# nishitbohra/RoViT-KAN-Interpretable-Vision-Transformer-for-Rose-Disease-Severity-Estimation

Measured on AMD Instinct MI355X. Metric: images/sec fwd+bwd, DeiT-Tiny+KAN 224^2, batch 256 per GPU, higher is better.
Workload: dtype bf16; 1 GPU; full RoViT-KAN (DeiT-Tiny + KAN + 3 heads) stage 4, train mode, batch 256/GPU, 224x224x3 randn images, random-init weights; step=fwd + JointLoss + bwd + grad all-reduce + clip_grad_norm(1.0) + AdamW, global_batch=256, parallelism=dp1, grad_buckets=2, rccl_world=0

## Files before the change

### include/rovit_hip.h

```cpp
#ifndef ROVIT_HIP_H
#define ROVIT_HIP_H

#include <stddef.h>
#include <stdint.h>

#ifdef __cplusplus
extern "C" {
#endif

typedef void* rovit_stream_t;

enum {
  ROVIT_OK = 0,
  ROVIT_ERR_SHAPE = -1,
  ROVIT_ERR_ALIGN = -2,
  ROVIT_ERR_NULL = -3,
  ROVIT_ERR_LAUNCH = -4
};

enum { ROVIT_ACT_NONE = 0, ROVIT_ACT_RELU = 1, ROVIT_ACT_SIGMOID3 = 2 };
enum { ROVIT_LIN_RELU = 1, ROVIT_LIN_CLAMP10 = 2 };
enum { ROVIT_EPI_BF16 = 0, ROVIT_EPI_GELU = 1, ROVIT_EPI_RESID = 2, ROVIT_EPI_MUL = 3, ROVIT_EPI_PATCH = 4 };
enum { ROVIT_GEMM_TILED_192 = 0x100, ROVIT_GEMM_TILED_96 = 0x200 };

// ... 133 lines not shown
                        float* rstd_out, float eps, rovit_stream_t stream);
size_t rovit_mlp_stream_bytes(void);
int rovit_mlp_prepare_stream(const void* w1f, const void* w2, void* wstream, rovit_stream_t stream);
int rovit_mlp_fused_fwd(const void* xhat2, const void* wstream, const float* b1, const float* b2, void* act, void* dact, float* X,
                        void* xhat_out, float* rstd_out, float eps, int M, int act_rows, rovit_stream_t stream);
int rovit_mlp_prepare_stream_tail(const void* w1f, const void* w2, const void* wproj, const void* wqkv_next, void* wstream,
                                  rovit_stream_t stream);
int rovit_block_tail_fwd(const void* o, const void* wstream, const float* bp, const float* b1, const float* b2, float* X, void* xhat2,
                         float* rstd2, void* act, void* dact, void* xhat_out, float* rstd_out, const float* bq_next, void* qkv_next,
                         float eps, int M, int act_rows, rovit_stream_t stream);
int rovit_mlp_fused_bwd(const void* dY, const void* wstream_bwd, const void* dact, void* dpre, const void* xhat2, const float* rstd2,
                        float* dX, void* dXb, int M, rovit_stream_t stream);
int rovit_mlp_prepare_stream_bwd(const void* w2T, const void* w1T, const void* wqkvT_next, void* wstream, rovit_stream_t stream);
int rovit_block_bwd_fused(const void* dqkv, const void* xhat1, const float* rstd1, const void* xmid_in, void* xout, const void* wstream_bwd,
                          const void* dact, void* dpre, const void* xhat2, const float* rstd2, void* dXb, int M, rovit_stream_t stream);
int rovit_gemm_ln_bwd(const void* dY, int ldy, const void* W, int ldw, int M, int K, const void* xhat, const float* rstd, float* dX,
                      const void* dXb_in, void* dXb, rovit_stream_t stream);
int rovit_wgrad_splits(int M, int N, int K);
size_t rovit_wgrad_workspace_bytes(int N, int K, int splits);
int rovit_wgrad(const void* dY, int ldy, const void* A, int lda, int M, int N, int K, int splits, int patch_tokens, float* ws,
                rovit_stream_t stream);
int rovit_wgrad_multi(const void* const* dY, const int* ldy, const void* const* A, const int* lda, const int* N, const int* K,
                      float* const* ws, int n, int M, int splits, rovit_stream_t stream);
int rovit_wgrad_multi_ex(const void* const* dY, const int* ldy, const void* const* A, const int* lda, const int* N, const int* K,
                         float* const* ws, const int* a_blk, const int* y_blk, int n, int M, int splits, rovit_stream_t stream);
int rovit_wgrad_reduce(const float* ws, int splits, int N, int K, const float* gamma, const float* beta, const float* W,
                       float* dW, float* db, float* dgamma, float* dbeta, float* g_scratch, rovit_stream_t stream);
int rovit_attention_fwd(const void* qkv, void* out, float* lse2, int batch, int tokens, int heads, int head_dim, float scale,
                        rovit_stream_t stream);
int rovit_attention_probs(const void* qkv, float* probs, int batch, int tokens, int heads, int head_dim, float scale,
                          rovit_stream_t stream);
int rovit_attention_bwd(const void* qkv, const void* out, const float* lse2, const void* dout, void* dqkv, int batch, int tokens,
// ... 363 lines not shown
```

### rovit-kan-interpretable-vision-transformer-for-rose-disease-severity-estimation_amd/csrc/common.h

```cpp
#pragma once
#include <hip/hip_runtime.h>
#include <stdint.h>
#include <stdio.h>

#include "../../include/rovit_hip.h"

typedef __bf16 bf16;
typedef __attribute__((ext_vector_type(8))) __bf16 bf16x8;
typedef __attribute__((ext_vector_type(4))) __bf16 bf16x4;
typedef __attribute__((ext_vector_type(4))) float f32x4;
typedef __attribute__((ext_vector_type(2))) float f32x2;

#define ROVIT_WAVE 64

void rovit_set_error(const char* fmt, ...);

#define ROVIT_CHECK_ARG(cond, code, ...)        \
  do {                                          \
    if (!(cond)) {                              \
      rovit_set_error(__VA_ARGS__);             \
      return (code);                            \
    }                                           \
  } while (0)

// ... 22 lines not shown
  ROVIT_KNOB_MLP_DBG = 7,
  ROVIT_KNOB_MLP_SCHEDULE = 8,
  ROVIT_KNOB_MLP_RPW = 9,
  ROVIT_KNOB_WGRAD_TILE = 10,
  ROVIT_KNOB_WGRAD_WGS = 11,
  ROVIT_KNOB_KAN_MFMA_NS = 12,
  ROVIT_KNOB_KDMA = 13,
  ROVIT_KNOB_SKIP_DX_FP32_STORE = 15,
  ROVIT_KNOB_SIDE_PRIORITY = 16,
  ROVIT_KNOB_PROJ_DGRAD_CUS = 17,
  ROVIT_KNOB_TAIL_WAVES = 18,
  ROVIT_KNOB_FWD_STAGGER = 19,
  ROVIT_KNOB_ATTN_FWD3 = 20,
  ROVIT_KNOB_GRADCAM_RECOMPUTE = 21,
  ROVIT_KNOB_SKIP_WGRAD_REDUCE = 14,
  ROVIT_KNOB_COUNT = 32
};
#ifdef ROVIT_DEV
extern int g_rovit_knob[ROVIT_KNOB_COUNT];
extern bool g_rovit_knob_set[ROVIT_KNOB_COUNT];
#define ROVIT_KNOB(id, dflt) (g_rovit_knob_set[id] ? g_rovit_knob[id] : (dflt))
#else
#define ROVIT_KNOB(id, dflt) (dflt)
#endif

#ifdef __HIPCC__

__device__ __forceinline__ f32x4 mfma16(bf16x8 a, bf16x8 b, f32x4 c) {
  return __builtin_amdgcn_mfma_f32_16x16x32_bf16(a, b, c, 0, 0, 0);
}
// ... 103 lines not shown
                       const int* targets, float* logits, int* chosen, float* dfeat, const float* wqkv, void* wt, int batch,
                       rovit_stream_t stream);
int rovit_gradcam_cam(const void* dqkv, const void* wt, const void* xhat1, const float* gamma, const float* beta, float* g, double* spart,
                      float* act, float* grad, float* cam, int batch, rovit_stream_t stream);
int rovit_gather_token_rows(const float* img_tokens, const float* base_tokens, int n_img, int base_shared, const int* seq_img, const int* src,
                            float* X, int n_seq, int tokens, rovit_stream_t stream);
int rovit_gradcam_wt(const float* wqkv, void* wt, rovit_stream_t stream);
int rovit_cls_tail_fwd(const void* o, float* X, const void* wproj, const float* bproj, const void* wfc1, const float* bfc1, const void* wfc2,
                       const float* bfc2, const float* gamma, const float* beta, void* xhat2, float* rstd2, void* act, void* dact, float* feat,
                       float* xhat_cls, float* rstd_cls, int rows, int tokens, float eps, rovit_stream_t stream);
int rovit_cls_tail_bwd(const float* dfeat, const float* xhat_cls, const float* rstd_cls, const float* gamma, const void* wfc2, const void* wfc1,
                       const void* wproj, const void* dact, const void* xhat2, const float* rstd2, void* xin, void* dpre, void* xmid, void* dO,
                       int rows, int tokens, rovit_stream_t stream);
int rovit_attention_bwd_rows(const void* qkv, const void* out, const float* lse2, const void* dout, int dout_rows, void* dqkv, int batch,
                             int tokens, int heads, int head_dim, float scale, rovit_stream_t stream);
int rovit_gemm_ln_bwd_cls(const void* dY, int ldy, const void* W, int ldw, int M, int K, const void* xhat, const float* rstd,
                          const void* dXb_in, int cls_step, void* dXb, rovit_stream_t stream);
struct RovitWgradDesc { const void* dY; int ldy; const void* A; int lda; int N, K; float* ws; int a_blk, y_blk; };
int rovit_wgrad_batch(const RovitWgradDesc* descs, int n, int M, int splits, rovit_stream_t stream);

struct RovitReduceDesc {
  const float* ws; int splits, N, K;
  const float* gamma; const float* beta; const float* W;
  float* dW; float* db; float* dgamma; float* dbeta; float* g_scratch;
};
int rovit_mlp_stream_prep_blocks(const void* prep_base, size_t blk0, size_t stride, size_t off_w1, size_t off_w2, size_t off_out,
                                 size_t off_wp, int bwd, size_t off_wq_next, int depth, rovit_stream_t stream, bool gelu_tables = true);
constexpr int ROVIT_REDUCE_BATCH = 4;
int rovit_wgrad_reduce_batch(const RovitReduceDesc* descs, int n, rovit_stream_t stream);
```

### rovit-kan-interpretable-vision-transformer-for-rose-disease-severity-estimation_amd/csrc/gemm.hip

```cpp
#include <cstdlib>
#include <type_traits>
#include "common.h"

#ifdef ROVIT_DEV
#define GEMM_DBG(g, bit) ((g).dbg & (bit))
#define GEMM_SET_DBG(g, v) (g).dbg = (v)
#else
#define GEMM_DBG(g, bit) (false)
#define GEMM_SET_DBG(g, v) ((void)0)
#endif

namespace {

inline bool set_max_lds(const void* fn, size_t bytes) { return rovit_set_max_lds(fn, bytes); }

constexpr int BK = 64;
constexpr int LDS_STRIDE = BK + 16;

enum { EPI_BF16 = 0, EPI_GELU = 1, EPI_RESID = 2, EPI_MUL = 3, EPI_PATCH = 4, EPI_RESID_LN = 5, EPI_LNBWD = 6,
       EPI_PATCH_IMG = 7 };

struct GemmArgs {
  const bf16* A; int lda;
  const bf16* W; int ldw;
// ... 1497 lines not shown
  ROVIT_CHECK_ARG(descs && n >= 1 && n <= WG_MAXPROB && M > 0 && splits > 0, ROVIT_ERR_SHAPE, "wgrad_batch: bad arguments");
  WgradArgs g{};
  g.nprob = n;
  for (int j = 0; j < n; ++j) {
    const RovitWgradDesc& d = descs[j];
    ROVIT_CHECK_ARG(d.dY && d.A && d.ws, ROVIT_ERR_NULL, "wgrad_batch: null pointer");
    ROVIT_CHECK_ARG(d.N % 96 == 0 && d.K % 192 == 0, ROVIT_ERR_SHAPE, "wgrad_batch: unsupported shape N=%d K=%d", d.N, d.K);
    ROVIT_CHECK_ARG(d.ldy % 8 == 0 && d.lda % 8 == 0 && rovit_aligned16(d.dY) && rovit_aligned16(d.A), ROVIT_ERR_ALIGN, "wgrad_batch: alignment");
    ROVIT_CHECK_ARG(!(d.a_blk && d.K % 32) && !(d.y_blk && d.N % 32), ROVIT_ERR_SHAPE, "wgrad_batch: chunk-major operands need 32-column chunks");
    g.p[j] = WgradProb{(const bf16*)d.dY, d.ldy, (const bf16*)d.A, d.lda, d.N, d.K, d.ws, d.ws + (size_t)splits * d.N * d.K, 0, 0, d.a_blk, d.y_blk};
  }
  g.M = M;
  g.splits = splits;
  g.rows_per_split = ((M + splits - 1) / splits + WG_MSTEP - 1) / WG_MSTEP * WG_MSTEP;
  GEMM_SET_DBG(g, ROVIT_KNOB(ROVIT_KNOB_GEMM_DBG, 0) >> 4);
  if (n == 1 && g.p[0].K % 96 == 0) launch_wgrad<96, 96>(g, (hipStream_t)stream);
  else {
    for (int j = 0; j < n; ++j) ROVIT_CHECK_ARG(descs[j].N % 192 == 0 && descs[j].K % 192 == 0, ROVIT_ERR_SHAPE, "wgrad_batch: N, K %% 192 for 192-wide tiles");
    launch_wgrad<192, 192, 4>(g, (hipStream_t)stream);
  }
  ROVIT_CHECK_LAUNCH("wgrad_kernel (batch)");
  return ROVIT_OK;
}

extern "C" int rovit_wgrad_multi(const void* const* dY, const int* ldy, const void* const* A, const int* lda, const int* N, const int* K,
                                 float* const* ws, int n, int M, int splits, rovit_stream_t stream) {
  ROVIT_CHECK_ARG(dY && ldy && A && lda && N && K && ws && n >= 1 && n <= WG_MAXPROB, ROVIT_ERR_NULL, "wgrad_multi: bad arguments");
  RovitWgradDesc d[WG_MAXPROB];
  for (int j = 0; j < n; ++j) d[j] = {dY[j], ldy[j], A[j], lda[j], N[j], K[j], ws[j]};
  return rovit_wgrad_batch(d, n, M, splits, stream);
}
// ... 59 lines not shown
  GemmArgs g{};
  g.A = (const bf16*)A; g.lda = lda; g.W = (const bf16*)W; g.ldw = ldw; g.M = M; g.N = 192; g.K = K; g.bias = bias;
  g.xres = X; g.ldx = 192; g.out = (bf16*)xhat_out; g.ldo = 192; g.rstd_out = rstd_out; g.eps = eps; GEMM_SET_DBG(g, ROVIT_KNOB(ROVIT_KNOB_GEMM_DBG, 0));
  if (K == 192) return launch_ws<6, 1, 64>(g, EPI_RESID_LN, (hipStream_t)stream);
  if (kdma_enabled() && xhat_out && K == 576) return launch_kdma<18, EPI_RESID_LN>(g, (hipStream_t)stream);
  if (K == 576) return launch_ws<9, 2, 32>(g, EPI_RESID_LN, (hipStream_t)stream);
  return launch_ws<12, 2, 32>(g, EPI_RESID_LN, (hipStream_t)stream);
}

static int gemm_ln_bwd_impl(const void* dY, int ldy, const void* W, int ldw, int M, int K, const void* xhat, const float* rstd,
                            float* dX, const void* dXb_in, int cls_step, void* dXb, rovit_stream_t stream);
extern "C" int rovit_gemm_ln_bwd(const void* dY, int ldy, const void* W, int ldw, int M, int K, const void* xhat, const float* rstd,
                                 float* dX, const void* dXb_in, void* dXb, rovit_stream_t stream) {
  return gemm_ln_bwd_impl(dY, ldy, W, ldw, M, K, xhat, rstd, dX, dXb_in, 0, dXb, stream);
}
int rovit_gemm_ln_bwd_cls(const void* dY, int ldy, const void* W, int ldw, int M, int K, const void* xhat, const float* rstd,
                          const void* dXb_in, int cls_step, void* dXb, rovit_stream_t stream) {
  ROVIT_CHECK_ARG(dXb_in && cls_step > 0, ROVIT_ERR_NULL, "gemm_ln_bwd_cls: needs the bf16 incoming gradient and a row step");
  return gemm_ln_bwd_impl(dY, ldy, W, ldw, M, K, xhat, rstd, nullptr, dXb_in, cls_step, dXb, stream);
}
static int gemm_ln_bwd_impl(const void* dY, int ldy, const void* W, int ldw, int M, int K, const void* xhat, const float* rstd,
                            float* dX, const void* dXb_in, int cls_step, void* dXb, rovit_stream_t stream) {
  ROVIT_CHECK_ARG(dY && W && xhat && rstd && (dX || dXb_in) && dXb, ROVIT_ERR_NULL, "gemm_ln_bwd: null pointer");
  ROVIT_CHECK_ARG(rovit_aligned16(dXb_in) && rovit_aligned16(dXb), ROVIT_ERR_ALIGN, "gemm_ln_bwd: alignment");
  ROVIT_CHECK_ARG(M > 0 && (K == 192 || K == 576 || K == 768), ROVIT_ERR_SHAPE, "gemm_ln_bwd: K must be 192/576/768 (got %d)", K);
  ROVIT_CHECK_ARG(ldy % 8 == 0 && ldw % 8 == 0 && rovit_aligned16(dY) && rovit_aligned16(W) && rovit_aligned16(dX), ROVIT_ERR_ALIGN,
                  "gemm_ln_bwd: alignment");
  GemmArgs g{};
  g.A = (const bf16*)dY; g.lda = ldy; g.W = (const bf16*)W; g.ldw = ldw; g.M = M; g.N = 192; g.K = K;
  g.mul = (const bf16*)xhat; g.ldm = 192; g.pos = rstd; g.xres = dX; g.ldx = 192; g.out = (bf16*)dXb; g.ldo = 192; g.xprev = (const bf16*)dXb_in; g.tokens = cls_step; GEMM_SET_DBG(g, ROVIT_KNOB(ROVIT_KNOB_GEMM_DBG, 0) | (ROVIT_KNOB(ROVIT_KNOB_SKIP_DX_FP32_STORE, 0) ? 64 : 0));
  if (K == 192) return launch_ws<6, 1, 64>(g, EPI_LNBWD, (hipStream_t)stream);
  if (kdma_enabled() && K == 576) return launch_kdma<18, EPI_LNBWD>(g, (hipStream_t)stream);
// ... 4 lines not shown
```

### rovit-kan-interpretable-vision-transformer-for-rose-disease-severity-estimation_amd/csrc/mlp_fused.hip

```cpp
#include <cstdlib>
#include "common.h"

#ifndef ROVIT_ACT_STORE_AUX
#define ROVIT_ACT_STORE_AUX 0
#endif
#ifndef ROVIT_MLP_PIPE_HINTS
#define ROVIT_MLP_PIPE_HINTS 0
#endif
#ifndef ROVIT_MLP_PIPE_SKEW
#define ROVIT_MLP_PIPE_SKEW 1
#endif

#ifdef ROVIT_DEV
#define MLP_DBG(g, bit) ((g).dbg & (bit))
#else
#define MLP_DBG(g, bit) (false)
#endif

namespace {

constexpr int D = 192, HID = 768, HC = 32, NCHUNK = HID / HC;
constexpr int PIECE = 512;
constexpr int CH_PIECES = 24;
constexpr int CH_ELEMS = CH_PIECES * PIECE;
// ... 29 lines not shown
  int act_rows;
  int rpw;
  const float* bp;
  bf16* dO;
  const float* bq;
  bf16* qkv;
  bf16* xhat2;
  float* rstd2;
  const bf16* gelu_table;
  const bf16* fw;
  const bf16* fdq;
  const bf16* fxhat;
  const float* frstd;
  const bf16* fxmid;
  bf16* fxout;
  float* X;
  bf16* xhat;
  float* rstd;
  bf16* xb;
  float eps;
  int M;
#ifdef ROVIT_DEV
  int dbg;
#endif
};

typedef unsigned int u32x4v __attribute__((ext_vector_type(4)));
typedef bf16 bf16x2 __attribute__((ext_vector_type(2)));

template <int N>
// ... 151 lines not shown
    barrier_lds();
#pragma unroll
    for (int p = 0; p < 4; ++p) ffetch(4 + p, pb[p], hb[p], rb[p]);
    auto ffinish = [&](int pass, const bf16x4 (&ps)[3], const bf16x4 (&hs)[3], float rr) {
      const int row = pass * RP + prow;
      const int m = r0 + row;
      float v[12], h[12];
      float s1 = 0.f, s2 = 0.f;
#pragma unroll
      for (int i = 0; i < 3; ++i) {
        const bf16x4 t = *(const bf16x4*)(Cs + row * CSTR + 64 * i + 4 * c16);
#pragma unroll
        for (int e = 0; e < 4; ++e) { v[4 * i + e] = (float)t[e]; h[4 * i + e] = (float)hs[i][e]; s1 += v[4 * i + e]; s2 += v[4 * i + e] * h[4 * i + e]; }
      }
      const float c1 = wave_sum16(s1) * (1.f / 192.f), c2 = wave_sum16(s2) * (1.f / 192.f);
      bf16x4 bq[3];
#pragma unroll
      for (int i = 0; i < 3; ++i) {
        f32x4 x = {(float)ps[i][0], (float)ps[i][1], (float)ps[i][2], (float)ps[i][3]};
#pragma unroll
        for (int e = 0; e < 4; ++e) x[e] += rr * (v[4 * i + e] - c1 - h[4 * i + e] * c2);
        bq[i] = pack4(x);
      }
#pragma unroll
      for (int i = 0; i < 3; ++i) *(bf16x4*)(Cs + row * CSTR + 64 * i + 4 * c16) = bq[i];
      if (row < g.rpw && m < g.M) {
        bf16x4* bp = (bf16x4*)(g.fxout + (size_t)m * D);
#pragma unroll
        for (int i = 0; i < 3; ++i) bp[16 * i + c16] = bq[i];
      }
    };
#pragma unroll
    for (int p = 0; p < 4; ++p) ffinish(p, pa[p], ha[p], ra[p]);
#pragma unroll
// ... 986 lines not shown
                  ROVIT_ERR_ALIGN, "mlp_fused_bwd: buffers must be 16-byte aligned");
  MlpArgs g{};
  g.xin = (const bf16*)dY; g.wstream = (const bf16*)wstream_bwd; g.act = (bf16*)dpre; g.mul = (const bf16*)dact; g.X = dX;
  g.xhat = (bf16*)const_cast<void*>(xhat2); g.rstd = const_cast<float*>(rstd2); g.xb = (bf16*)dXb; g.M = M;
#ifdef ROVIT_DEV
  g.dbg = ROVIT_KNOB(ROVIT_KNOB_MLP_DBG, 0) | (ROVIT_KNOB(ROVIT_KNOB_SKIP_DX_FP32_STORE, 0) ? 64 : 0);
#endif
  ROVIT_CHECK_ARG(rovit_set_max_lds((const void*)mlp_fused_kernel<1, 1, 8>, lds_bytes(1, 8)), ROVIT_ERR_LAUNCH,
                  "mlp_fused_bwd: cannot raise the LDS limit");
  g.rpw = mlp_rpw(M);
  hipLaunchKernelGGL((mlp_fused_kernel<1, 1, 8>), dim3((M + g.rpw - 1) / g.rpw), dim3(512), lds_bytes(1, 8), (hipStream_t)stream, g);
  ROVIT_CHECK_LAUNCH("mlp_fused_kernel (backward)");
  return ROVIT_OK;
}

extern "C" int rovit_block_bwd_fused(const void* dqkv, const void* xhat1, const float* rstd1, const void* xmid_in, void* xout,
                                     const void* wstream_bwd, const void* dact, void* dpre, const void* xhat2, const float* rstd2,
                                     void* dXb, int M, rovit_stream_t stream) {
  if (!dqkv) return rovit_mlp_fused_bwd(xout, wstream_bwd, dact, dpre, xhat2, rstd2, nullptr, dXb, M, stream);
  ROVIT_CHECK_ARG(xhat1 && rstd1 && xmid_in && xout && wstream_bwd, ROVIT_ERR_NULL, "block_bwd_fused: null pointer");
  ROVIT_CHECK_ARG(!dact || (dpre && xhat2 && rstd2 && dXb), ROVIT_ERR_NULL, "block_bwd_fused: null pointer in the MLP part");
  ROVIT_CHECK_ARG(M > 0 && (size_t)M * HID * 2 < ((size_t)1 << 31), ROVIT_ERR_SHAPE, "block_bwd_fused: M = %d out of range", M);
  ROVIT_CHECK_ARG(rovit_aligned16(dqkv) && rovit_aligned16(xhat1) && rovit_aligned16(xmid_in) && rovit_aligned16(xout) &&
                      rovit_aligned16(wstream_bwd) && rovit_aligned16(dact) && rovit_aligned16(dpre) && rovit_aligned16(xhat2) &&
                      rovit_aligned16(dXb),
                  ROVIT_ERR_ALIGN, "block_bwd_fused: buffers must be 16-byte aligned");
  MlpArgs g{};
  g.fdq = (const bf16*)dqkv; g.fxhat = (const bf16*)xhat1; g.frstd = rstd1; g.fxmid = (const bf16*)xmid_in; g.fxout = (bf16*)xout;
  g.wstream = (const bf16*)wstream_bwd; g.fw = g.wstream + (size_t)FRONT_ENTRY0 * CH_ELEMS;
  g.act = (bf16*)dpre; g.mul = (const bf16*)dact; g.xhat = (bf16*)const_cast<void*>(xhat2); g.rstd = const_cast<float*>(rstd2);
  g.xb = (bf16*)dXb; g.M = M;
  ROVIT_CHECK_ARG(rovit_set_max_lds((const void*)mlp_fused_kernel<1, 1, 8, false, false, false, 2, true>, lds_bytes(1, 8)), ROVIT_ERR_LAUNCH,
                  "block_bwd_fused: cannot raise the LDS limit");
  g.rpw = mlp_rpw(M);
  hipLaunchKernelGGL((mlp_fused_kernel<1, 1, 8, false, false, false, 2, true>), dim3((M + g.rpw - 1) / g.rpw), dim3(512), lds_bytes(1, 8),
                     (hipStream_t)stream, g);
  ROVIT_CHECK_LAUNCH("mlp_fused_kernel (backward with the front phase)");
  return ROVIT_OK;
}

#ifdef ROVIT_DEV
extern "C" int rovit_block_tail_bwd(const void* dY, const void* wstream_bwd, const void* dact, void* dpre, const void* xhat2,
                                    const float* rstd2, float* dX, void* dXb, void* dO, int M, rovit_stream_t stream) {
  ROVIT_CHECK_ARG(dY && wstream_bwd && dact && dpre && xhat2 && rstd2 && dX && dXb, ROVIT_ERR_NULL, "block_tail_bwd: null pointer");
  ROVIT_CHECK_ARG(M > 0 && (size_t)M * HID * 2 < ((size_t)1 << 31), ROVIT_ERR_SHAPE, "block_tail_bwd: M = %d out of range", M);
  ROVIT_CHECK_ARG(rovit_aligned16(dY) && rovit_aligned16(wstream_bwd) && rovit_aligned16(dact) && rovit_aligned16(dpre) &&
                      rovit_aligned16(xhat2) && rovit_aligned16(dX) && rovit_aligned16(dXb) && rovit_aligned16(dO),
                  ROVIT_ERR_ALIGN, "block_tail_bwd: buffers must be 16-byte aligned");
  MlpArgs g{};
  g.xin = (const bf16*)dY; g.act = (bf16*)dpre; g.mul = (const bf16*)dact; g.X = dX; g.dO = (bf16*)dO;
  g.wstream = (const bf16*)wstream_bwd + (size_t)(NCHUNK + PENTRIES) * CH_ELEMS;
  g.xhat = (bf16*)const_cast<void*>(xhat2); g.rstd = const_cast<float*>(rstd2); g.xb = (bf16*)dXb; g.M = M;
#ifdef ROVIT_DEV
// ... 11 lines not shown
```

### rovit-kan-interpretable-vision-transformer-for-rose-disease-severity-estimation_amd/csrc/vit.hip

```cpp
#include <algorithm>
#include <vector>

#include "common.h"

namespace {

constexpr int T = 197, D = 192, H = 3, MLP = 768, PD = 768;
enum { EPI_BF16 = 0, EPI_GELU = 1, EPI_RESID = 2, EPI_MUL = 3, EPI_PATCH = 4 };
enum { P_CLS = 0, P_POS, P_PATCH_W, P_PATCH_B, P_NORM_W, P_NORM_B, P_BLOCK0 };
enum { B_N1W = 0, B_N1B, B_QKVW, B_QKVB, B_PROJW, B_PROJB, B_N2W, B_N2B, B_FC1W, B_FC1B, B_FC2W, B_FC2B, B_COUNT };

inline size_t al(size_t x) { return (x + 255) & ~(size_t)255; }

constexpr long MLP_FUSED_MIN_ROWS = 34000;
inline bool mlp_one_launch(int mlp_path, long rows) {
  return mlp_path == ROVIT_MLP_ONE_LAUNCH || (mlp_path == ROVIT_MLP_AUTO && rows >= MLP_FUSED_MIN_ROWS);
}

struct Prep {
  size_t wpe;
  size_t blk0, blk_stride;
  size_t wqkv, wqkvT, wproj, wprojT, wfc1, wfc1T, wfc2, wfc2T, bqkv, bfc1;
  size_t wmlp, wmlpb;
  size_t total;
// ... 525 lines not shown
  if (first_block == depth - 1) {
    ROVIT_CHECK_ARG(d_features, ROVIT_ERR_NULL, "vit_backward: null d_features");
  }
  hipStream_t sA = (hipStream_t)stream;
  SideStream* ss = (wgrad && two_streams_enabled()) ? side_stream() : nullptr;
  hipStream_t sB = ss ? ss->stream : sA;
  static hipEvent_t no_events[64];
  if (ss && !(ss->carry && first_block != depth - 1)) {
    ss->next = 0;
    for (auto& e : ss->ev_bdone) e = nullptr;
  }
  if (ss) ss->carry = false;
  hipEvent_t* ev_bdone = ss ? ss->ev_bdone : no_events;
  int pending = -1;
  int a5_pending = -1;
#define EVFAIL(what) do { rovit_set_error("vit_backward: " what " failed"); return ROVIT_ERR_LAUNCH; } while (0)
  const int S_MERGE = std::min(std::min(ROVIT_KNOB(ROVIT_KNOB_WGRAD_SPLITS, 16), L.s_fc1), std::min(std::min(L.s_fc2, L.s_qkv), L.s_proj));
  ROVIT_CHECK_ARG(S_MERGE >= 1, ROVIT_ERR_SHAPE, "vit_backward: no weight-gradient split fits batch %d", batch);
  auto qkv_reduce_desc = [&](int i, int splits) -> RovitReduceDesc {
    const float* const* bp = params + P_BLOCK0 + B_COUNT * i;
    float* const* bg = grads + P_BLOCK0 + B_COUNT * i;
    return {(const float*)(ws + L.slab_qkv), splits, 3 * D, D, bp[B_N1W], bp[B_N1B], bp[B_QKVW], bg[B_QKVW], bg[B_QKVB], bg[B_N1W],
            bg[B_N1B], (float*)(ws + L.gscr2)};
  };
  auto issue_qkv = [&](int i) -> int {
    char* s = ws + L.blk0 + (size_t)i * L.blk_stride;
    const RovitWgradDesc wd = {ws + L.dqkv[i & 1], 3 * D, s + L.xhat1, D, 3 * D, D, (float*)(ws + L.slab_qkv)};
    RUN(rovit_wgrad_batch(&wd, 1, M, S_MERGE, sB));
    const RovitReduceDesc rd = qkv_reduce_desc(i, S_MERGE);
    RUN(rovit_wgrad_reduce_batch(&rd, 1, sB));
    if (ss && !(ev_bdone[i] = hand_over(ss, sB, nullptr, true))) EVFAIL("event record");
    return ROVIT_OK;
  };
  auto issue_merged = [&](int i, int prev, const char* xin, const char* dp, const char* xmid) -> int {
    char* s = ws + L.blk0 + (size_t)i * L.blk_stride;
    const float* const* bp = params + P_BLOCK0 + B_COUNT * i;
    float* const* bg = grads + P_BLOCK0 + B_COUNT * i;
    RovitWgradDesc wd[4];
    RovitReduceDesc rd[4];
    int n = 0;
    const int blk = one_launch ? 1 : 0;
    wd[n] = {xin, D, s + L.act, MLP, D, MLP, (float*)(ws + L.slab_fc2), blk, 0};
    rd[n++] = {(const float*)(ws + L.slab_fc2), S_MERGE, D, MLP, nullptr, nullptr, nullptr, bg[B_FC2W], bg[B_FC2B], nullptr, nullptr, nullptr};
    wd[n] = {dp, MLP, s + L.xhat2, D, MLP, D, (float*)(ws + L.slab_fc1), 0, blk};
    rd[n++] = {(const float*)(ws + L.slab_fc1), S_MERGE, MLP, D, bp[B_N2W], bp[B_N2B], bp[B_FC1W], bg[B_FC1W], bg[B_FC1B], bg[B_N2W], bg[B_N2B],
               (float*)(ws + L.gscr)};
    wd[n] = {xmid, D, s + L.o, D, D, D, (float*)(ws + L.slab_proj)};
    rd[n++] = {(const float*)(ws + L.slab_proj), S_MERGE, D, D, nullptr, nullptr, nullptr, bg[B_PROJW], bg[B_PROJB], nullptr, nullptr, nullptr};
    if (prev >= 0) {
      char* sp = ws + L.blk0 + (size_t)prev * L.blk_stride;
      wd[n] = {ws + L.dqkv[prev & 1], 3 * D, sp + L.xhat1, D, 3 * D, D, (float*)(ws + L.slab_qkv)};
      rd[n++] = qkv_reduce_desc(prev, S_MERGE);
    }
    RUN(rovit_wgrad_batch(wd, n, M, S_MERGE, sB));
    RUN(rovit_wgrad_reduce_batch(rd, n, sB));
    if (prev >= 0 && ss && !(ev_bdone[prev] = hand_over(ss, sB, nullptr, true))) EVFAIL("event record");
    return ROVIT_OK;
  };
  for (int i = first_block; i >= last_block; --i) {
    const char* q = pb + P.blk0 + (size_t)i * P.blk_stride;
    char* s = ws + L.blk0 + (size_t)i * L.blk_stride;
    char* xin = x0v(i);
    char* xout = x0v(i - 1);
    if (i == depth - 1) {
      const int Mr = batch, rs = T;
      char* dp = ws + L.dpre[i & 1];
      char* dq = ws + L.dqkv[i & 1];
      char* xmc = ws + L.x1[i & 1];
      RUN(rovit_cls_tail_bwd(d_features, (const float*)(ws + L.xhat_cls), (const float*)(ws + L.rstd_cls), params[P_NORM_W], q + P.wfc2, q + P.wfc1,
                             q + P.wproj, s + L.dact, s + L.xhat2, (const float*)(s + L.rstd2), xin, dp, xmc, ws + L.dO, batch, T, stream));
      if (rel) {
        RUN(rovit_attention_relevance_step(s + L.qkv, (const float*)(s + L.lse), ws + L.dO, rel->u, rel->scratch, batch, 1, stream));
        if (i == 0) break;
      }
      if (ss && !hand_over(ss, sA, sB)) EVFAIL("event hand-over");
      if (wgrad) RUN(rovit_cls_norm_affine_grad(d_features, (const float*)(ws + L.xhat_cls), grads[P_NORM_W], grads[P_NORM_B], batch, sB));
      if (wgrad) {
        const float* const* bpp = params + P_BLOCK0 + B_COUNT * i;
        float* const* bg = grads + P_BLOCK0 + B_COUNT * i;
        const int sc = std::min(std::min(4, L.s_fc2c), std::min(L.s_fc1c, L.s_projc));
        const RovitWgradDesc wd[3] = {{xin, D * rs, s + L.act, MLP * rs, D, MLP, (float*)(ws + L.slab_fc2)},
                                      {dp, MLP * rs, s + L.xhat2, D * rs, MLP, D, (float*)(ws + L.slab_fc1)},
                                      {xmc, D * rs, s + L.o, D * rs, D, D, (float*)(ws + L.slab_proj)}};
        RUN(rovit_wgrad_batch(wd, 3, Mr, sc, sB));
        const RovitReduceDesc rd[3] = {
            {(const float*)(ws + L.slab_fc2), sc, D, MLP, nullptr, nullptr, nullptr, bg[B_FC2W], bg[B_FC2B], nullptr, nullptr, nullptr},
            {(const float*)(ws + L.slab_fc1), sc, MLP, D, bpp[B_N2W], bpp[B_N2B], bpp[B_FC1W], bg[B_FC1W], bg[B_FC1B], bg[B_N2W], bg[B_N2B],
             (float*)(ws + L.gscr)},
            {(const float*)(ws + L.slab_proj), sc, D, D, nullptr, nullptr, nullptr, bg[B_PROJW], bg[B_PROJB], nullptr, nullptr, nullptr}};
        RUN(rovit_wgrad_reduce_batch(rd, 3, sB));
      }
      RUN(rovit_attention_cls_bwd(s + L.qkv, s + L.o, (const float*)(s + L.lse), ws + L.dO, dq, batch, T, H, D / H, 0.125f, stream));
      RUN(rovit_gemm_ln_bwd_cls(dq, 3 * D, q + P.wqkvT, 3 * D, M, 3 * D, s + L.xhat1, (const float*)(s + L.rstd1), xmc, T, xout, stream));
      pending = i;
      continue;
    }
    const int p = i & 1;
    char* dp = ws + L.dpre[p];
    char* dq = ws + L.dqkv[p];
    char* xmid = ws + L.x1[p];
    const bool wait_b = ss && i + 2 < depth && ev_bdone[i + 2];
    const bool wait_early = i + 3 >= depth;
    if (wait_b && wait_early && hipStreamWaitEvent(sA, ev_bdone[i + 2], 0) != hipSuccess) EVFAIL("event wait");
    if (one_launch && a5_pending == i + 1) {
      char* su = ws + L.blk0 + (size_t)(i + 1) * L.blk_stride;
      RUN(rovit_block_bwd_fused(ws + L.dqkv[(i + 1) & 1], su + L.xhat1, (const float*)(su + L.rstd1), ws + L.x1[(i + 1) & 1], xin, q + P.wmlpb,
                                s + L.dact, dp, s + L.xhat2, (const float*)(s + L.rstd2), xmid, M, sA));
      a5_pending = -1;
    } else if (one_launch) {
      RUN(rovit_mlp_fused_bwd(xin, q + P.wmlpb, s + L.dact, dp, s + L.xhat2, (const float*)(s + L.rstd2), nullptr, xmid, M, sA));
    } else {
      RUN(rovit_gemm_nt(xin, D, q + P.wfc2T, D, M, MLP, D, nullptr, EPI_MUL, dp, MLP, nullptr, nullptr, 0, s + L.dact, MLP, nullptr, 0, sA));
      RUN(rovit_gemm_ln_bwd(dp, MLP, q + P.wfc1T, MLP, M, MLP, s + L.xhat2, (const float*)(s + L.rstd2), nullptr, xin, xmid, sA));
    }
    if (ss && !hand_over(ss, sA, sB)) EVFAIL("event hand-over");
    if (wgrad) RUN(issue_merged(i, pending, xin, dp, xmid));
    {
      const int cus = ROVIT_KNOB(ROVIT_KNOB_PROJ_DGRAD_CUS, 256);
      if (cus != 256) rovit_set_cu_budget(cus);
      const int rc_a3 = rovit_gemm_nt(xmid, D, q + P.wprojT, D, M, D, D, nullptr, EPI_BF16, ws + L.dO, D, nullptr, nullptr, 0, nullptr, 0, nullptr, 0,
                                      sA);
      if (cus != 256) rovit_set_cu_budget(256);
      if (rc_a3 != ROVIT_OK) return rc_a3;
    }
    if (rel) {
      RUN(rovit_attention_relevance_step(s + L.qkv, (const float*)(s + L.lse), ws + L.dO, rel->u, rel->scratch, batch, 0, sA));
      if (i == 0) break;
    }
    if (wait_b && !wait_early && hipStreamWaitEvent(sA, ev_bdone[i + 2], 0) != hipSuccess) EVFAIL("event wait");
    RUN(rovit_attention_bwd(s + L.qkv, s + L.o, (const float*)(s + L.lse), ws + L.dO, dq, batch, T, H, D / H, 0.125f, sA));
    if (one_launch && i > last_block) {
      a5_pending = i;
    } else if (one_launch && i > 0) {
      RUN(rovit_block_bwd_fused(dq, s + L.xhat1, (const float*)(s + L.rstd1), xmid, xout, q - P.blk_stride + P.wmlpb, nullptr, nullptr, nullptr,
                                nullptr, nullptr, M, sA));
    } else {
      RUN(rovit_gemm_ln_bwd(dq, 3 * D, q + P.wqkvT, 3 * D, M, 3 * D, s + L.xhat1, (const float*)(s + L.rstd1), nullptr, xmid, xout, sA));
    }
    pending = i;
  }
  auto patch_grads = [&]() -> int {
    ROVIT_CHECK_ARG(images, ROVIT_ERR_NULL, "vit_backward: the range ending at block 0 needs the images of the forward call");
    RUN(rovit_patch_embed_wgrad(x0v(-1), D, images, batch, T, D, L.s_pe, (float*)(ws + L.slab_pe), stream));
    RUN(rovit_wgrad_reduce((const float*)(ws + L.slab_pe), L.s_pe, D, PD, nullptr, nullptr, nullptr, grads[P_PATCH_W], grads[P_PATCH_B],
                           nullptr, nullptr, nullptr, stream));
    RUN(rovit_pos_grad(nullptr, x0v(-1), grads[P_POS], grads[P_CLS], batch, T, stream));
    return ROVIT_OK;
  };
  auto pixel_grads = [&]() -> int {
    if (!d_images) return ROVIT_OK;
    return rovit_patch_embed_dgrad(x0v(-1), D, pb + P.wpe, d_images, batch / ig->copies, ig->copies, ig->scale, ig->accumulate, stream);
  };
  bool patch_done = false;
  if (pending >= 0 && wgrad) {
    if (ss && !hand_over(ss, sA, sB)) EVFAIL("event hand-over");
    RUN(issue_qkv(pending));
    if (ss && last_block == 0) { RUN(patch_grads()); RUN(pixel_grads()); patch_done = true; }
    if (ss && defer_join && last_block > 0) {
      if (!hand_over(ss, sB, notify)) EVFAIL("event hand-over");
      ss->carry = true;
    } else if (ss && !hand_over(ss, sB, sA)) {
      EVFAIL("event hand-over");
    }
  }
#undef EVFAIL
  if (last_block == 0 && !patch_done) {
    if (wgrad) RUN(patch_grads());
    RUN(pixel_grads());
  }
  return ROVIT_OK;
}
// ... 32 lines not shown
```

### rovit-kan-interpretable-vision-transformer-for-rose-disease-severity-estimation_amd/rovit_hip/native.py

```python
from __future__ import annotations

import ctypes as C
import os
from typing import Optional, Sequence

import torch

_PKG_ROOT = os.path.dirname(os.path.dirname(os.path.abspath(__file__)))
LIB_PATH = os.environ.get('ROVIT_HIP_LIB') or os.path.join(_PKG_ROOT, 'lib', 'librovit_hip.so')

_lib: Optional[C.CDLL] = None
ABI_VERSION = 440

_vp, _i, _f, _sz = C.c_void_p, C.c_int, C.c_float, C.c_size_t

MLP_AUTO, MLP_TWO_LAUNCH, MLP_ONE_LAUNCH = 0, 1, 2
GEMM_TILED_192, GEMM_TILED_96 = 0x100, 0x200
MLP_FUSED_MIN_ROWS = 34000

SIGNATURES = {
    'rovit_version': (_i, []),
    'rovit_last_error_string': (C.c_char_p, []),
    'rovit_kan_basis': (_i, [_vp, _vp, _vp, _i, _i, _vp]),
    'rovit_kan_layer_fwd': (_i, [_vp] * 6 + [_i] * 5 + [_vp]),
# ... 37 lines not shown
    'rovit_vit_backward_input': (_i, [_vp] * 6 + [_i] * 5 + [_vp] + [_vp, _i, _f, _i]),
    'rovit_vit_backward_relevance': (_i, [_vp] * 4 + [_i] * 3 + [_vp] * 3),
    'rovit_attention_relevance_step': (_i, [_vp] * 5 + [_i, _i, _vp]),
    'rovit_vit_embed': (_i, [_vp] * 4 + [_i, _i, _vp]),
    'rovit_vit_forward_tokens': (_i, [_vp, _vp, _i, _i, _vp, _vp, _i] + [_vp] * 4 + [_i, _i, _i, _vp]),
    'rovit_gemm_nt': (_i, [_vp, _i, _vp, _i, _i, _i, _i, _vp, _i, _vp, _i, _vp, _vp, _i, _vp, _i, _vp, _i, _vp]),
    'rovit_gemm_resid_ln': (_i, [_vp, _i, _vp, _i, _i, _i, _vp, _vp, _vp, _vp, _f, _vp]),
    'rovit_mlp_stream_bytes': (_sz, []),
    'rovit_mlp_prepare_stream': (_i, [_vp, _vp, _vp, _vp]),
    'rovit_mlp_fused_fwd': (_i, [_vp] * 9 + [_f, _i, _i, _vp]),
    'rovit_mlp_prepare_stream_tail': (_i, [_vp] * 6),
    'rovit_block_tail_fwd': (_i, [_vp] * 14 + [_f, _i, _i, _vp]),
    'rovit_mlp_fused_bwd': (_i, [_vp] * 8 + [_i, _vp]),
    'rovit_mlp_prepare_stream_bwd': (_i, [_vp] * 5),
    'rovit_block_bwd_fused': (_i, [_vp] * 11 + [_i, _vp]),
    'rovit_gemm_ln_bwd': (_i, [_vp, _i, _vp, _i, _i, _i, _vp, _vp, _vp, _vp, _vp, _vp]),
    'rovit_wgrad_splits': (_i, [_i, _i, _i]),
    'rovit_wgrad_workspace_bytes': (_sz, [_i, _i, _i]),
    'rovit_wgrad': (_i, [_vp, _i, _vp, _i, _i, _i, _i, _i, _i, _vp, _vp]),
    'rovit_wgrad_multi': (_i, [_vp] * 7 + [_i, _i, _i, _vp]),
    'rovit_wgrad_multi_ex': (_i, [_vp] * 9 + [_i, _i, _i, _vp]),
    'rovit_wgrad_reduce': (_i, [_vp, _i, _i, _i] + [_vp] * 8 + [_vp]),
    'rovit_attention_fwd': (_i, [_vp, _vp, _vp, _i, _i, _i, _i, _f, _vp]),
    'rovit_attention_bwd': (_i, [_vp] * 5 + [_i] * 4 + [_f, _vp]),
    'rovit_attention_cls_fwd': (_i, [_vp, _vp, _vp, _i, _i, _i, _i, _f, _vp]),
    'rovit_attention_cls_bwd': (_i, [_vp] * 5 + [_i] * 4 + [_f, _vp]),
    'rovit_layernorm_fwd': (_i, [_vp, _vp, _vp, _i, _i, _f, _vp]),
    'rovit_layernorm_bwd': (_i, [_vp] * 5 + [_i, _i, _vp]),
    'rovit_im2col': (_i, [_vp, _vp, _i, _vp]),
    'rovit_patch_embed_fwd': (_i, [_vp, _vp, _vp, _vp, _vp, _i, _i, _vp]),
# ... 335 lines not shown
```

Baseline: 64250 images/sec.

## Fuse CLS-block dgrad into next fused block backward and release qkv wgrad early

Adds a strided-input variant of the fused block backward so the last block's CLS-only LN/qkv dgrad is folded into the next block's fused kernel rather than launched separately. It also moves the final block's qkv weight-gradient issue on the side stream earlier, before the bottom dgrad. It can run the CLS attention backward before the side-stream wgrad work and cap the CU budget of the bottom gemm_ln_bwd so the side-stream work overlaps it. Risks include added per-row branching in the kernel and contention between the two streams.

Result: faster. 65170 images/sec, median of 6 (+1.4%).

```diff
diff --git a/include/rovit_hip.h b/include/rovit_hip.h
--- a/include/rovit_hip.h
+++ b/include/rovit_hip.h
@@ -171,8 +171,13 @@
 int rovit_mlp_prepare_stream_bwd(const void* w2T, const void* w1T, const void* wqkvT_next, void* wstream, rovit_stream_t stream);
 int rovit_block_bwd_fused(const void* dqkv, const void* xhat1, const float* rstd1, const void* xmid_in, void* xout, const void* wstream_bwd,
                           const void* dact, void* dpre, const void* xhat2, const float* rstd2, void* dXb, int M, rovit_stream_t stream);
+int rovit_block_bwd_fused_cls(const void* dqkv, const void* xhat1, const float* rstd1, const void* xmid_in, int xmid_step, void* xout,
+                              const void* wstream_bwd, const void* dact, void* dpre, const void* xhat2, const float* rstd2, void* dXb, int M,
+                              rovit_stream_t stream);
 int rovit_gemm_ln_bwd(const void* dY, int ldy, const void* W, int ldw, int M, int K, const void* xhat, const float* rstd, float* dX,
                       const void* dXb_in, void* dXb, rovit_stream_t stream);
+int rovit_gemm_ln_bwd_cls(const void* dY, int ldy, const void* W, int ldw, int M, int K, const void* xhat, const float* rstd,
+                          const void* dXb_in, int cls_step, void* dXb, rovit_stream_t stream);
 int rovit_wgrad_splits(int M, int N, int K);
 size_t rovit_wgrad_workspace_bytes(int N, int K, int splits);
 int rovit_wgrad(const void* dY, int ldy, const void* A, int lda, int M, int N, int K, int splits, int patch_tokens, float* ws,
diff --git a/rovit-kan-interpretable-vision-transformer-for-rose-disease-severity-estimation_amd/csrc/common.h b/rovit-kan-interpretable-vision-transformer-for-rose-disease-severity-estimation_amd/csrc/common.h
--- a/rovit-kan-interpretable-vision-transformer-for-rose-disease-severity-estimation_amd/csrc/common.h
+++ b/rovit-kan-interpretable-vision-transformer-for-rose-disease-severity-estimation_amd/csrc/common.h
@@ -60,6 +60,9 @@
   ROVIT_KNOB_ATTN_FWD3 = 20,
   ROVIT_KNOB_GRADCAM_RECOMPUTE = 21,
   ROVIT_KNOB_SKIP_WGRAD_REDUCE = 14,
+  ROVIT_KNOB_BWD_ENDS = 22,
+  ROVIT_KNOB_BOTTOM_A5_CUS = 23,
+  ROVIT_KNOB_LONE_WGRAD_192 = 24,
   ROVIT_KNOB_COUNT = 32
 };
 #ifdef ROVIT_DEV
@@ -193,8 +196,6 @@
                        int rows, int tokens, rovit_stream_t stream);
 int rovit_attention_bwd_rows(const void* qkv, const void* out, const float* lse2, const void* dout, int dout_rows, void* dqkv, int batch,
                              int tokens, int heads, int head_dim, float scale, rovit_stream_t stream);
-int rovit_gemm_ln_bwd_cls(const void* dY, int ldy, const void* W, int ldw, int M, int K, const void* xhat, const float* rstd,
-                          const void* dXb_in, int cls_step, void* dXb, rovit_stream_t stream);
 struct RovitWgradDesc { const void* dY; int ldy; const void* A; int lda; int N, K; float* ws; int a_blk, y_blk; };
 int rovit_wgrad_batch(const RovitWgradDesc* descs, int n, int M, int splits, rovit_stream_t stream);
 
diff --git a/rovit-kan-interpretable-vision-transformer-for-rose-disease-severity-estimation_amd/csrc/gemm.hip b/rovit-kan-interpretable-vision-transformer-for-rose-disease-severity-estimation_amd/csrc/gemm.hip
--- a/rovit-kan-interpretable-vision-transformer-for-rose-disease-severity-estimation_amd/csrc/gemm.hip
+++ b/rovit-kan-interpretable-vision-transformer-for-rose-disease-severity-estimation_amd/csrc/gemm.hip
@@ -1535,7 +1535,7 @@
   g.splits = splits;
   g.rows_per_split = ((M + splits - 1) / splits + WG_MSTEP - 1) / WG_MSTEP * WG_MSTEP;
   GEMM_SET_DBG(g, ROVIT_KNOB(ROVIT_KNOB_GEMM_DBG, 0) >> 4);
-  if (n == 1 && g.p[0].K % 96 == 0) launch_wgrad<96, 96>(g, (hipStream_t)stream);
+  if (n == 1 && g.p[0].K % 96 == 0 && !ROVIT_KNOB(ROVIT_KNOB_LONE_WGRAD_192, 0)) launch_wgrad<96, 96>(g, (hipStream_t)stream);
   else {
     for (int j = 0; j < n; ++j) ROVIT_CHECK_ARG(descs[j].N % 192 == 0 && descs[j].K % 192 == 0, ROVIT_ERR_SHAPE, "wgrad_batch: N, K %% 192 for 192-wide tiles");
     launch_wgrad<192, 192, 4>(g, (hipStream_t)stream);
@@ -1625,8 +1625,8 @@
                                  float* dX, const void* dXb_in, void* dXb, rovit_stream_t stream) {
   return gemm_ln_bwd_impl(dY, ldy, W, ldw, M, K, xhat, rstd, dX, dXb_in, 0, dXb, stream);
 }
-int rovit_gemm_ln_bwd_cls(const void* dY, int ldy, const void* W, int ldw, int M, int K, const void* xhat, const float* rstd,
-                          const void* dXb_in, int cls_step, void* dXb, rovit_stream_t stream) {
+extern "C" int rovit_gemm_ln_bwd_cls(const void* dY, int ldy, const void* W, int ldw, int M, int K, const void* xhat, const float* rstd,
+                                     const void* dXb_in, int cls_step, void* dXb, rovit_stream_t stream) {
   ROVIT_CHECK_ARG(dXb_in && cls_step > 0, ROVIT_ERR_NULL, "gemm_ln_bwd_cls: needs the bf16 incoming gradient and a row step");
   return gemm_ln_bwd_impl(dY, ldy, W, ldw, M, K, xhat, rstd, nullptr, dXb_in, cls_step, dXb, stream);
 }
diff --git a/rovit-kan-interpretable-vision-transformer-for-rose-disease-severity-estimation_amd/csrc/mlp_fused.hip b/rovit-kan-interpretable-vision-transformer-for-rose-disease-severity-estimation_amd/csrc/mlp_fused.hip
--- a/rovit-kan-interpretable-vision-transformer-for-rose-disease-severity-estimation_amd/csrc/mlp_fused.hip
+++ b/rovit-kan-interpretable-vision-transformer-for-rose-disease-severity-estimation_amd/csrc/mlp_fused.hip
@@ -67,6 +67,7 @@
   const float* frstd;
   const bf16* fxmid;
   bf16* fxout;
+  int fstep;
   float* X;
   bf16* xhat;
   float* rstd;
@@ -248,10 +249,11 @@
         for (int e = 0; e < 4; ++e) { v[4 * i + e] = (float)t[e]; h[4 * i + e] = (float)hs[i][e]; s1 += v[4 * i + e]; s2 += v[4 * i + e] * h[4 * i + e]; }
       }
       const float c1 = wave_sum16(s1) * (1.f / 192.f), c2 = wave_sum16(s2) * (1.f / 192.f);
+      const bool has_in = g.fstep <= 0 || (m % g.fstep) == 0;
       bf16x4 bq[3];
 #pragma unroll
       for (int i = 0; i < 3; ++i) {
-        f32x4 x = {(float)ps[i][0], (float)ps[i][1], (float)ps[i][2], (float)ps[i][3]};
+        f32x4 x = has_in ? (f32x4){(float)ps[i][0], (float)ps[i][1], (float)ps[i][2], (float)ps[i][3]} : (f32x4){0.f, 0.f, 0.f, 0.f};
 #pragma unroll
         for (int e = 0; e < 4; ++e) x[e] += rr * (v[4 * i + e] - c1 - h[4 * i + e] * c2);
         bq[i] = pack4(x);
@@ -1268,9 +1270,10 @@
   return ROVIT_OK;
 }
 
-extern "C" int rovit_block_bwd_fused(const void* dqkv, const void* xhat1, const float* rstd1, const void* xmid_in, void* xout,
-                                     const void* wstream_bwd, const void* dact, void* dpre, const void* xhat2, const float* rstd2,
-                                     void* dXb, int M, rovit_stream_t stream) {
+static int block_bwd_fused_impl(const void* dqkv, const void* xhat1, const float* rstd1, const void* xmid_in, int xmid_step, void* xout,
+                                const void* wstream_bwd, const void* dact, void* dpre, const void* xhat2, const float* rstd2,
+                                void* dXb, int M, rovit_stream_t stream) {
+  ROVIT_CHECK_ARG(xmid_step >= 0, ROVIT_ERR_SHAPE, "block_bwd_fused: xmid_step must be >= 0, got %d", xmid_step);
   if (!dqkv) return rovit_mlp_fused_bwd(xout, wstream_bwd, dact, dpre, xhat2, rstd2, nullptr, dXb, M, stream);
   ROVIT_CHECK_ARG(xhat1 && rstd1 && xmid_in && xout && wstream_bwd, ROVIT_ERR_NULL, "block_bwd_fused: null pointer");
   ROVIT_CHECK_ARG(!dact || (dpre && xhat2 && rstd2 && dXb), ROVIT_ERR_NULL, "block_bwd_fused: null pointer in the MLP part");
@@ -1281,6 +1284,7 @@
                   ROVIT_ERR_ALIGN, "block_bwd_fused: buffers must be 16-byte aligned");
   MlpArgs g{};
   g.fdq = (const bf16*)dqkv; g.fxhat = (const bf16*)xhat1; g.frstd = rstd1; g.fxmid = (const bf16*)xmid_in; g.fxout = (bf16*)xout;
+  g.fstep = xmid_step;
   g.wstream = (const bf16*)wstream_bwd; g.fw = g.wstream + (size_t)FRONT_ENTRY0 * CH_ELEMS;
   g.act = (bf16*)dpre; g.mul = (const bf16*)dact; g.xhat = (bf16*)const_cast<void*>(xhat2); g.rstd = const_cast<float*>(rstd2);
   g.xb = (bf16*)dXb; g.M = M;
@@ -1291,6 +1295,16 @@
                      (hipStream_t)stream, g);
   ROVIT_CHECK_LAUNCH("mlp_fused_kernel (backward with the front phase)");
   return ROVIT_OK;
+}
+extern "C" int rovit_block_bwd_fused(const void* dqkv, const void* xhat1, const float* rstd1, const void* xmid_in, void* xout,
+                                     const void* wstream_bwd, const void* dact, void* dpre, const void* xhat2, const float* rstd2,
+                                     void* dXb, int M, rovit_stream_t stream) {
+  return block_bwd_fused_impl(dqkv, xhat1, rstd1, xmid_in, 0, xout, wstream_bwd, dact, dpre, xhat2, rstd2, dXb, M, stream);
+}
+extern "C" int rovit_block_bwd_fused_cls(const void* dqkv, const void* xhat1, const float* rstd1, const void* xmid_in, int xmid_step,
+                                         void* xout, const void* wstream_bwd, const void* dact, void* dpre, const void* xhat2,
+                                         const float* rstd2, void* dXb, int M, rovit_stream_t stream) {
+  return block_bwd_fused_impl(dqkv, xhat1, rstd1, xmid_in, xmid_step, xout, wstream_bwd, dact, dpre, xhat2, rstd2, dXb, M, stream);
 }
 
 #ifdef ROVIT_DEV
diff --git a/rovit-kan-interpretable-vision-transformer-for-rose-disease-severity-estimation_amd/csrc/vit.hip b/rovit-kan-interpretable-vision-transformer-for-rose-disease-severity-estimation_amd/csrc/vit.hip
--- a/rovit-kan-interpretable-vision-transformer-for-rose-disease-severity-estimation_amd/csrc/vit.hip
+++ b/rovit-kan-interpretable-vision-transformer-for-rose-disease-severity-estimation_amd/csrc/vit.hip
@@ -563,6 +563,10 @@
   hipEvent_t* ev_bdone = ss ? ss->ev_bdone : no_events;
   int pending = -1;
   int a5_pending = -1;
+  const int ends = ROVIT_KNOB(ROVIT_KNOB_BWD_ENDS, 11);
+  const bool cls_fuse = (ends & 1) != 0, early_release = (ends & 2) != 0, a4_early = (ends & 8) != 0;
+  const bool serial_bottom = (ends & 4) != 0 && last_block == 0;
+  bool flushed = false;
 #define EVFAIL(what) do { rovit_set_error("vit_backward: " what " failed"); return ROVIT_ERR_LAUNCH; } while (0)
   const int S_MERGE = std::min(std::min(ROVIT_KNOB(ROVIT_KNOB_WGRAD_SPLITS, 16), L.s_fc1), std::min(std::min(L.s_fc2, L.s_qkv), L.s_proj));
   ROVIT_CHECK_ARG(S_MERGE >= 1, ROVIT_ERR_SHAPE, "vit_backward: no weight-gradient split fits batch %d", batch);
@@ -575,10 +579,11 @@
   auto issue_qkv = [&](int i) -> int {
     char* s = ws + L.blk0 + (size_t)i * L.blk_stride;
     const RovitWgradDesc wd = {ws + L.dqkv[i & 1], 3 * D, s + L.xhat1, D, 3 * D, D, (float*)(ws + L.slab_qkv)};
-    RUN(rovit_wgrad_batch(&wd, 1, M, S_MERGE, sB));
+    hipStream_t sQ = serial_bottom ? sA : sB;
+    RUN(rovit_wgrad_batch(&wd, 1, M, S_MERGE, sQ));
     const RovitReduceDesc rd = qkv_reduce_desc(i, S_MERGE);
-    RUN(rovit_wgrad_reduce_batch(&rd, 1, sB));
-    if (ss && !(ev_bdone[i] = hand_over(ss, sB, nullptr, true))) EVFAIL("event record");
+    RUN(rovit_wgrad_reduce_batch(&rd, 1, sQ));
+    if (ss && !(ev_bdone[i] = hand_over(ss, sQ, nullptr, true))) EVFAIL("event record");
     return ROVIT_OK;
   };
   auto issue_merged = [&](int i, int prev, const char* xin, const char* dp, const char* xmid) -> int {
@@ -606,6 +611,13 @@
     if (prev >= 0 && ss && !(ev_bdone[prev] = hand_over(ss, sB, nullptr, true))) EVFAIL("event record");
     return ROVIT_OK;
   };
+  auto release_early = [&](int i) -> int {
+    if (!(early_release && !serial_bottom && ss && wgrad && i == last_block)) return ROVIT_OK;
+    if (!hand_over(ss, sA, sB)) EVFAIL("event hand-over");
+    RUN(issue_qkv(i));
+    flushed = true;
+    return ROVIT_OK;
+  };
   for (int i = first_block; i >= last_block; --i) {
     const char* q = pb + P.blk0 + (size_t)i * P.blk_stride;
     char* s = ws + L.blk0 + (size_t)i * L.blk_stride;
@@ -623,6 +635,8 @@
         if (i == 0) break;
       }
       if (ss && !hand_over(ss, sA, sB)) EVFAIL("event hand-over");
+      const bool a4_first = ss && a4_early;
+      if (a4_first) RUN(rovit_attention_cls_bwd(s + L.qkv, s + L.o, (const float*)(s + L.lse), ws + L.dO, dq, batch, T, H, D / H, 0.125f, stream));
       if (wgrad) RUN(rovit_cls_norm_affine_grad(d_features, (const float*)(ws + L.xhat_cls), grads[P_NORM_W], grads[P_NORM_B], batch, sB));
       if (wgrad) {
         const float* const* bpp = params + P_BLOCK0 + B_COUNT * i;
@@ -639,8 +653,13 @@
             {(const float*)(ws + L.slab_proj), sc, D, D, nullptr, nullptr, nullptr, bg[B_PROJW], bg[B_PROJB], nullptr, nullptr, nullptr}};
         RUN(rovit_wgrad_reduce_batch(rd, 3, sB));
       }
-      RUN(rovit_attention_cls_bwd(s + L.qkv, s + L.o, (const float*)(s + L.lse), ws + L.dO, dq, batch, T, H, D / H, 0.125f, stream));
-      RUN(rovit_gemm_ln_bwd_cls(dq, 3 * D, q + P.wqkvT, 3 * D, M, 3 * D, s + L.xhat1, (const float*)(s + L.rstd1), xmc, T, xout, stream));
+      if (!a4_first) RUN(rovit_attention_cls_bwd(s + L.qkv, s + L.o, (const float*)(s + L.lse), ws + L.dO, dq, batch, T, H, D / H, 0.125f, stream));
+      if (one_launch && cls_fuse && i > last_block) {
+        a5_pending = i;
+      } else {
+        RUN(release_early(i));
+        RUN(rovit_gemm_ln_bwd_cls(dq, 3 * D, q + P.wqkvT, 3 * D, M, 3 * D, s + L.xhat1, (const float*)(s + L.rstd1), xmc, T, xout, stream));
+      }
       pending = i;
       continue;
     }
@@ -653,8 +672,9 @@
     if (wait_b && wait_early && hipStreamWaitEvent(sA, ev_bdone[i + 2], 0) != hipSuccess) EVFAIL("event wait");
     if (one_launch && a5_pending == i + 1) {
       char* su = ws + L.blk0 + (size_t)(i + 1) * L.blk_stride;
-      RUN(rovit_block_bwd_fused(ws + L.dqkv[(i + 1) & 1], su + L.xhat1, (const float*)(su + L.rstd1), ws + L.x1[(i + 1) & 1], xin, q + P.wmlpb,
-                                s + L.dact, dp, s + L.xhat2, (const float*)(s + L.rstd2), xmid, M, sA));
+      RUN(rovit_block_bwd_fused_cls(ws + L.dqkv[(i + 1) & 1], su + L.xhat1, (const float*)(su + L.rstd1), ws + L.x1[(i + 1) & 1],
+                                    i + 1 == depth - 1 ? T : 0, xin, q + P.wmlpb, s + L.dact, dp, s + L.xhat2, (const float*)(s + L.rstd2),
+                                    xmid, M, sA));
       a5_pending = -1;
     } else if (one_launch) {
       RUN(rovit_mlp_fused_bwd(xin, q + P.wmlpb, s + L.dact, dp, s + L.xhat2, (const float*)(s + L.rstd2), nullptr, xmid, M, sA));
@@ -678,13 +698,19 @@
     }
     if (wait_b && !wait_early && hipStreamWaitEvent(sA, ev_bdone[i + 2], 0) != hipSuccess) EVFAIL("event wait");
     RUN(rovit_attention_bwd(s + L.qkv, s + L.o, (const float*)(s + L.lse), ws + L.dO, dq, batch, T, H, D / H, 0.125f, sA));
+    RUN(release_early(i));
     if (one_launch && i > last_block) {
       a5_pending = i;
     } else if (one_launch && i > 0) {
       RUN(rovit_block_bwd_fused(dq, s + L.xhat1, (const float*)(s + L.rstd1), xmid, xout, q - P.blk_stride + P.wmlpb, nullptr, nullptr, nullptr,
                                 nullptr, nullptr, M, sA));
     } else {
-      RUN(rovit_gemm_ln_bwd(dq, 3 * D, q + P.wqkvT, 3 * D, M, 3 * D, s + L.xhat1, (const float*)(s + L.rstd1), nullptr, xmid, xout, sA));
+      const int cus = flushed ? ROVIT_KNOB(ROVIT_KNOB_BOTTOM_A5_CUS, 160) : 256;
+      if (cus != 256) rovit_set_cu_budget(cus);
+      const int rc_a5 = rovit_gemm_ln_bwd(dq, 3 * D, q + P.wqkvT, 3 * D, M, 3 * D, s + L.xhat1, (const float*)(s + L.rstd1), nullptr, xmid, xout,
+                                          sA);
+      if (cus != 256) rovit_set_cu_budget(256);
+      if (rc_a5 != ROVIT_OK) return rc_a5;
     }
     pending = i;
   }
@@ -702,8 +728,10 @@
   };
   bool patch_done = false;
   if (pending >= 0 && wgrad) {
-    if (ss && !hand_over(ss, sA, sB)) EVFAIL("event hand-over");
-    RUN(issue_qkv(pending));
+    if (!flushed) {
+      if (ss && !hand_over(ss, sA, sB)) EVFAIL("event hand-over");
+      RUN(issue_qkv(pending));
+    }
     if (ss && last_block == 0) { RUN(patch_grads()); RUN(pixel_grads()); patch_done = true; }
     if (ss && defer_join && last_block > 0) {
       if (!hand_over(ss, sB, notify)) EVFAIL("event hand-over");
diff --git a/rovit-kan-interpretable-vision-transformer-for-rose-disease-severity-estimation_amd/rovit_hip/native.py b/rovit-kan-interpretable-vision-transformer-for-rose-disease-severity-estimation_amd/rovit_hip/native.py
--- a/rovit-kan-interpretable-vision-transformer-for-rose-disease-severity-estimation_amd/rovit_hip/native.py
+++ b/rovit-kan-interpretable-vision-transformer-for-rose-disease-severity-estimation_amd/rovit_hip/native.py
@@ -75,6 +75,8 @@
     'rovit_mlp_fused_bwd': (_i, [_vp] * 8 + [_i, _vp]),
     'rovit_mlp_prepare_stream_bwd': (_i, [_vp] * 5),
     'rovit_block_bwd_fused': (_i, [_vp] * 11 + [_i, _vp]),
+    'rovit_block_bwd_fused_cls': (_i, [_vp] * 4 + [_i] + [_vp] * 7 + [_i, _vp]),
+    'rovit_gemm_ln_bwd_cls': (_i, [_vp, _i, _vp, _i, _i, _i, _vp, _vp, _vp, _i, _vp, _vp]),
     'rovit_gemm_ln_bwd': (_i, [_vp, _i, _vp, _i, _i, _i, _vp, _vp, _vp, _vp, _vp, _vp]),
     'rovit_wgrad_splits': (_i, [_i, _i, _i]),
     'rovit_wgrad_workspace_bytes': (_sz, [_i, _i, _i]),
```
